# UCL-CCS/SCEMa

Hardware: AMD Instinct MI355X
Metric: stress_evals_per_sec (higher is better)
Workload: dtype f64; 1 GPU; 576 x PE-10368 OPLS replicas per update(), 10+100 MD steps each (dt 2 fs, 300 K, lj/cut/coul/long 12/9 + PPPM 1e-4 + SHAKE + NVT), persistent per-QP state, replica equilibrated for 2000 steps before the timed region; force_field=opls, strain_set=balanced (load/unload: odd updates take the draw with the opposite sign), n_sims=576, atoms_per_replica=10368, sims_on_rank0=576, allgathers=0

## Files before the change

### include/scema_md.h

```cpp
#ifndef SCEMA_MD_H
#define SCEMA_MD_H

#include <stdint.h>

#ifdef __cplusplus
extern "C" {
#endif

#define SCEMA_MD_OK 0
#define SCEMA_MD_ERR_ARG 1
#define SCEMA_MD_ERR_NOSTATE 2
#define SCEMA_MD_ERR_DEVICE 3
#define SCEMA_MD_ERR_BOX 4
#define SCEMA_MD_ERR_IO 5
#define SCEMA_MD_ERR_OVERFLOW 6

#define SCEMA_MD_NPART 8
#define SCEMA_MD_QP_NONE ((int32_t)0xFFFFFFFF)

typedef struct scema_md_engine scema_md_engine;

typedef struct {
  double cut_lj;
  double cut_coul;
// ... 142 lines not shown
                           double length[3], double stress[6], double stiff[36]);

typedef struct {
  int32_t nsteps_equil;
  double timestep_length;
  double temperature;
  int64_t seed;
} scema_md_equilparams;
int scema_md_equilibrate(scema_md_engine *e, const char *matid, int32_t replica, const scema_md_equilparams *p, double length[3],
                         double *info);

int scema_md_debug_minimize(scema_md_engine *e, int32_t qp_id, const char *matid, int32_t replica, double etol, double ftol,
                            int32_t maxiter, int32_t maxeval, double *info);
int scema_md_debug_run_nh(scema_md_engine *e, int32_t qp_id, const char *matid, int32_t replica, int32_t nsteps, double dt,
                          double t_start, double t_stop, int32_t npt, double p_target, double p_period, double *lavg);
int scema_md_debug_compute(scema_md_engine *e, int32_t qp_id, const char *matid, int32_t replica, int32_t use_shake,
                           double *f, double *energies, double *virials, double *info );
int scema_md_debug_skin_bands(scema_md_engine *e, int32_t pos, uint64_t *out, int32_t cap);
int scema_md_debug_rows(scema_md_engine *e, int32_t pos, int32_t *cnt, int32_t *rows, int64_t rows_cap, int32_t *info);
int scema_md_debug_run(scema_md_engine *e, int32_t qp_id, const char *matid, int32_t replica, int32_t nsteps,
                       double dt, double temperature, int32_t nvt, int32_t use_shake, const double *rates,
                       double *press_avg);

int scema_md_reax_configure(scema_md_engine *e, const char *ffield_path, const char *const *elements, int32_t n_elements,
                            double qeq_tol, double skin);
int scema_md_reax_activate(scema_md_engine *e, int32_t on);
int scema_md_reax_set(scema_md_engine *e, int32_t exact_gradient, int32_t terms, int32_t qeq_maxiter);
int scema_md_reax_concurrency(scema_md_engine *e, int32_t halves, int32_t overlap);
int scema_md_batch_split(scema_md_engine *e, int32_t on);
int scema_md_get_concurrency(const scema_md_engine *e, int32_t *out);
int scema_md_pppm_tiling(scema_md_engine *e, int32_t mode, int32_t lds_bytes);
int scema_md_pppm_binning(scema_md_engine *e, int32_t mode);
long long scema_md_pppm_binned_launches(const scema_md_engine *e);
int scema_md_pppm_paths(const scema_md_engine *e, int32_t out[8]);
int scema_md_pppm_tile_shape(const int32_t grid[3], int32_t lds_bytes, int32_t which , int32_t out[4]);
int scema_md_pppm_plan_count(const scema_md_engine *e);
int scema_md_reax_debug_compute(scema_md_engine *e, int32_t qp_id, const char *matid, int32_t replica, double *f, double *eparts,
                                double *virial, double *q, double *info);
int scema_md_reax_stats(const scema_md_engine *e, double *out);

int scema_md_sw_configure(scema_md_engine *e, const char *matid, const char *sw_path, const char *const *elements, int32_t n_elements,
                          int32_t energy_unit, double skin);
int scema_md_sw_debug_compute(scema_md_engine *e, int32_t qp_id, const char *matid, int32_t replica, double *f, double *e2, double *e3,
                              double *virial, double *info);
int scema_md_sw_read_params(const char *sw_path, const char *const *elements, int32_t n_elements, int32_t energy_unit, int32_t *n_kept,
                            int32_t *type_map, double *values, char *errbuf, int32_t errcap);

int scema_md_tersoff_configure(scema_md_engine *e, const char *matid, const char *path, const char *const *elements, int32_t n_elements,
                               int32_t energy_unit, double skin);
int scema_md_tersoff_debug_compute(scema_md_engine *e, int32_t qp_id, const char *matid, int32_t replica, double *f, double *e_rep,
                                   double *e_att, double *virial, double *info);
int scema_md_tersoff_read_params(const char *path, const char *const *elements, int32_t n_elements, int32_t energy_unit, int32_t *n_kept,
                                 int32_t *type_map, double *values, char *errbuf, int32_t errcap);

int scema_md_tersoff_mod_configure(scema_md_engine *e, const char *matid, const char *path, const char *const *elements, int32_t n_elements,
                                   int32_t energy_unit, double skin);
int scema_md_tersoff_mod_debug_compute(scema_md_engine *e, int32_t qp_id, const char *matid, int32_t replica, double *f, double *e_rep,
                                       double *e_att, double *virial, double *info);
int scema_md_tersoff_zbl_configure(scema_md_engine *e, const char *matid, const char *path, const char *const *elements, int32_t n_elements,
                                   int32_t energy_unit, double skin);
int scema_md_tersoff_zbl_debug_compute(scema_md_engine *e, int32_t qp_id, const char *matid, int32_t replica, double *f, double *e_rep,
                                       double *e_att, double *virial, double *info);
int scema_md_tersoff_mod_read_params(const char *path, const char *const *elements, int32_t n_elements, int32_t energy_unit, int32_t *n_kept,
                                     int32_t *type_map, double *values, char *errbuf, int32_t errcap);
int scema_md_tersoff_zbl_read_params(const char *path, const char *const *elements, int32_t n_elements, int32_t energy_unit, int32_t *n_kept,
                                     int32_t *type_map, double *values, char *errbuf, int32_t errcap);
// ... 89 lines not shown
```

### scema_amd/capi.py

```python
from __future__ import annotations

import ctypes as C
import os

import numpy as np

_HERE = os.path.dirname(os.path.abspath(__file__))
LIB_PATH = os.path.join(_HERE, os.environ.get("SCEMA_MD_LIB") or ("libscema_md_asan.so" if os.environ.get("SCEMA_SANITIZE") == "1" else "libscema_md.so"))

NPART = 8
PARTS = ["lj", "coul", "bond", "angle", "dihedral", "improper", "kspace", "shake"]
QP_NONE = -1

SYMBOLS = [
    "scema_md_default_params", "scema_md_create", "scema_md_destroy", "scema_md_last_error",
    "scema_md_register_replica", "scema_md_load_replica_file", "scema_md_write_replica_file",
    "scema_md_load_lammps_data", "scema_md_convert_lammps_data",
    "scema_md_probe_lammps_restart", "scema_md_read_lammps_restart_atoms", "scema_md_load_lammps_restart",
    "scema_md_convert_lammps_restart", "scema_md_write_lammps_restart",
    "scema_md_strain_batch", "scema_md_strain", "scema_md_local_stress_device_ptr",
    "scema_md_local_stress_count", "scema_md_local_result_doubles", "scema_md_copy_local_stress", "scema_md_scatter_gathered", "scema_md_settle_update", "scema_md_has_state", "scema_md_get_state",
    "scema_md_set_state", "scema_md_drop_state", "scema_md_save_state_file", "scema_md_load_state_file", "scema_md_save_state_lammps",
    "scema_md_init_material", "scema_md_debug_compute", "scema_md_debug_run", "scema_md_debug_skin_bands", "scema_md_debug_rows", "scema_md_get_profile", "scema_md_env_overrides",
    "scema_md_comm_unique_id", "scema_md_comm_init_rccl", "scema_md_comm_init_host", "scema_md_comm_destroy",
    "scema_md_comm_world", "scema_md_comm_rank", "scema_md_comm_stats", "scema_md_comm_handshakes", "scema_md_state_owner", "scema_md_last_plan",
    "scema_plan_dir_create", "scema_plan_dir_destroy", "scema_plan_update", "scema_md_kspace_setup",
    "scema_md_save_state_dump", "scema_md_replica_natoms", "scema_md_save_replica_file", "scema_md_equilibrate", "scema_md_debug_minimize", "scema_md_debug_run_nh",
    "scema_md_reax_configure", "scema_md_reax_activate", "scema_md_reax_set", "scema_md_reax_concurrency", "scema_md_batch_split", "scema_md_get_concurrency", "scema_md_pppm_plan_count", "scema_md_pppm_tiling", "scema_md_pppm_binning", "scema_md_pppm_binned_launches", "scema_md_pppm_paths", "scema_md_pppm_tile_shape", "scema_md_unsettled_updates", "scema_md_reax_debug_compute", "scema_md_reax_stats", "scema_md_box_fma_tflops",
    "scema_md_sw_configure", "scema_md_sw_debug_compute", "scema_md_sw_read_params",
    "scema_md_tersoff_configure", "scema_md_tersoff_debug_compute", "scema_md_tersoff_read_params",
    "scema_md_eam_configure", "scema_md_eam_debug_compute", "scema_md_eam_read_setfl",
    "scema_md_tersoff_mod_configure", "scema_md_tersoff_mod_debug_compute", "scema_md_tersoff_mod_read_params",
    "scema_md_tersoff_zbl_configure", "scema_md_tersoff_zbl_debug_compute", "scema_md_tersoff_zbl_read_params",
    "scema_md_vashishta_configure", "scema_md_vashishta_debug_compute", "scema_md_vashishta_read_params",
    "scema_md_adp_configure", "scema_md_adp_debug_compute", "scema_md_adp_read_setfl",
    "scema_md_edip_configure", "scema_md_edip_debug_compute", "scema_md_edip_read_params",
    "scema_md_meam_spline_configure", "scema_md_meam_spline_debug_compute", "scema_md_meam_spline_read_params", "scema_md_meam_spline_eval",
    "scema_md_born_dsf_configure", "scema_md_born_dsf_debug_compute", "scema_md_born_dsf_read_params", "scema_md_born_dsf_eval",
    "scema_md_born_long_configure", "scema_md_born_long_debug_compute", "scema_md_born_long_read_params", "scema_md_born_long_eval",
    "scema_md_born_long_kvectors",
]
COMM_ID_BYTES = 128
HOST_ALLGATHER_FN = C.CFUNCTYPE(C.c_int, C.c_void_p, C.c_void_p, C.c_void_p, C.c_int64)
HOST_SEND_FN = C.CFUNCTYPE(C.c_int, C.c_void_p, C.c_void_p, C.c_int64, C.c_int32)
HOST_RECV_FN = C.CFUNCTYPE(C.c_int, C.c_void_p, C.c_void_p, C.c_int64, C.c_int32)


class EquilParams(C.Structure):
    _fields_ = [("nsteps_equil", C.c_int32), ("timestep_length", C.c_double), ("temperature", C.c_double), ("seed", C.c_int64)]


class Params(C.Structure):
    _fields_ = [("cut_lj", C.c_double), ("cut_coul", C.c_double), ("skin", C.c_double), ("neigh_delay", C.c_int32),
                ("kspace_accuracy", C.c_double), ("shake_tol", C.c_double), ("shake_maxiter", C.c_int32),
                ("shake_mass", C.c_double), ("t_period", C.c_double), ("t_chain", C.c_int32), ("device", C.c_int32),
                ("max_batch", C.c_int32), ("profile", C.c_int32), ("kspace_style", C.c_int32)]


_P = C.c_void_p


# ... 365 lines not shown
        arr = (C.c_char_p * len(elements))(*[e.encode() for e in elements])
        self._chk(lib().scema_md_reax_configure(self.h, ffield.encode(), arr, C.c_int32(len(elements)), C.c_double(qeq_tol), C.c_double(skin)))

    def reax_activate(self, on: bool = True):
        self._chk(lib().scema_md_reax_activate(self.h, C.c_int32(1 if on else 0)))

    def reax_set(self, exact_gradient: int = -1, terms: int = -1, qeq_maxiter: int = -1):
        self._chk(lib().scema_md_reax_set(self.h, C.c_int32(exact_gradient), C.c_int32(terms), C.c_int32(qeq_maxiter)))

    def reax_concurrency(self, halves: int = -1, overlap: int = -1):
        self._chk(lib().scema_md_reax_concurrency(self.h, C.c_int32(halves), C.c_int32(overlap)))

    def unsettled_updates(self) -> int:
        lib().scema_md_unsettled_updates.restype = C.c_int64
        return int(lib().scema_md_unsettled_updates(self.h))

    def batch_split(self, on: int = -1):
        self._chk(lib().scema_md_batch_split(self.h, C.c_int32(on)))

    def pppm_plan_count(self) -> int:
        lib().scema_md_pppm_plan_count.restype = C.c_int
        return int(lib().scema_md_pppm_plan_count(self.h))

    def pppm_tiling(self, mode: int = -1, lds_bytes: int = -1):
        self._chk(lib().scema_md_pppm_tiling(self.h, C.c_int32(mode), C.c_int32(lds_bytes)))

    def pppm_binning(self, mode: int = -1):
        self._chk(lib().scema_md_pppm_binning(self.h, C.c_int32(mode)))

    def pppm_binned_launches(self) -> int:
        lib().scema_md_pppm_binned_launches.restype = C.c_longlong
        return int(lib().scema_md_pppm_binned_launches(self.h))

    def pppm_paths(self) -> dict:
        out = (C.c_int32 * 8)()
        self._chk(lib().scema_md_pppm_paths(self.h, out))
        return dict(spread=int(out[0]), force=int(out[1]), spread_tiles=(int(out[2]), int(out[3])), force_tiles=(int(out[4]), int(out[5])),
                    lds_bytes=int(out[6]), mode=int(out[7]))

    def concurrency(self) -> dict:
        out = (C.c_int32 * 3)()
        self._chk(lib().scema_md_get_concurrency(self.h, out))
        return dict(split=int(out[0]), reax_halves=int(out[1]), reax_overlap=int(out[2]))

    def reax_compute(self, matid, replica, qp=QP_NONE):
        n = self._natoms[(matid, replica)]
        f = np.zeros((n, 3)); e = np.zeros(len(REAX_PARTS)); w = np.zeros(6); q = np.zeros(n); info = np.zeros(6)
        self._chk(lib().scema_md_reax_debug_compute(self.h, C.c_int32(qp), matid.encode(), C.c_int32(replica), _p(f), _p(e), _p(w), _p(q), _p(info)))
        return dict(f=f, e=dict(zip(REAX_PARTS, e)), w=w, q=q, maxneigh_seen=int(info[0]), maxnb=int(info[1]), maxbd=int(info[2]),
                    qeq_iters=int(info[3]), image_search=int(info[4]), maxbonds_seen=int(info[5]))

    def _row_configure(self, symbol, matid, path, elements, energy_unit, skin):
        arr = (C.c_char_p * len(elements))(*[e.encode() for e in elements])
        self._chk(getattr(lib(), symbol)(self.h, matid.encode(), path.encode(), arr, C.c_int32(len(elements)), C.c_int32(energy_unit), C.c_double(skin)))

    def _row_compute(self, symbol, matid, replica, qp, ea_key, eb_key, count_key):
        n = self.natoms(matid, replica)
        f = np.zeros((n, 3)); ea = C.c_double(0.0); eb = C.c_double(0.0); w = np.zeros(6); info = np.zeros(4)
        self._chk(getattr(lib(), symbol)(self.h, C.c_int32(qp), matid.encode(), C.c_int32(replica), _p(f), C.byref(ea), C.byref(eb), _p(w), _p(info)))
        return {"f": f, ea_key: ea.value, eb_key: eb.value, "w": w, "maxrow": int(info[0]), "rowcap": int(info[1]), "npairs": int(info[2]),
                count_key: int(info[3])}

    def sw_configure(self, matid: str, sw_path: str, elements=("Si",), energy_unit: int = 0, skin: float = -1.0):
        self._row_configure("scema_md_sw_configure", matid, sw_path, elements, energy_unit, skin)

    def sw_compute(self, matid, replica, qp=QP_NONE):
# ... 433 lines not shown
```

### scema_amd/csrc/engine/engine.h

```cpp
#pragma once
#include <hip/hip_runtime.h>
#include <rccl/rccl.h>

#include <algorithm>
#include <cmath>
#include <cstdarg>
#include <cstdio>
#include <cstdlib>
#include <chrono>
#include <thread>
#include <cstring>
#include <ctime>
#include <array>
#include <atomic>
#include <functional>
#include <map>
#include <memory>
#include <sstream>
#include <fstream>
#include <string>
#include <vector>

#include "../../../include/scema_md.h"
#include "host/reax_ffield.h"
// ... 270 lines not shown
struct scema_md_engine {
  scema_md_params p;
  hipStream_t stream = nullptr;
  double skin_extra_fixed = 0.0;
  bool skin_adapt = false;
  hipStream_t stream2 = nullptr;
  hipStream_t stream3 = nullptr;
  hipEvent_t ev_up = nullptr;
  bool split_streams = true;
  hipEvent_t ev_fork = nullptr, ev_join = nullptr;
  bool rx_qeq_failed = false;
  long long rx_precond_fallbacks = 0;
  bool rx_precond = true;
  int rx_halves = 2, rx_overlap = 1;
  struct RxPart { hipStream_t main = nullptr, side = nullptr; hipEvent_t ev[4] = {nullptr, nullptr, nullptr, nullptr}; };
  std::vector<RxPart> rx_parts;
  std::vector<hipEvent_t> md_part_done;
  hipStream_t rx_side1 = nullptr;
  hipEvent_t rx_side1_ev[4] = {nullptr, nullptr, nullptr, nullptr};
  hipEvent_t row_fork = nullptr;
  std::map<std::string, std::unique_ptr<Topo>> topos;
  std::map<std::string, std::unique_ptr<State>> states;
  std::vector<std::unique_ptr<Slot>> slots;
  DevBuf d_sims, d_sc, d_local_stress, d_kpack, d_minptr, d_boxpair, d_pppm, d_copytab;
  std::vector<MdkCopy> h_copytab;
  DevBuf d_zerotab, d_rxstat;
  std::vector<MdkZero> h_zerotab;
  std::vector<long long> h_rxstat;
  std::vector<std::unique_ptr<DevBuf>> bak_x, bak_v;
  int pppm_tile_mode = 1, pppm_lds_bytes = 0;
  int pppm_paths[8] = {0, 0, 0, 0, 0, 0, 0, 1};
  int pppm_bin_mode = 2;
  long long pppm_binned_launches = 0;
  std::map<std::array<int, 6>, hipfftHandle> pppm_plans;
  std::vector<int> h_kpack;
  int local_stress_count = 0;
  std::vector<SimDev> h_sims;
  std::vector<SimScalars> h_sc;
  std::vector<hipEvent_t> ev_pool;
  Profile prof;
  std::string err;
  double neigh_grow = 1.0;
  double jtab_grow = 1.0;
  int overflow_bits = 0;
  double overflow_need_j = 1.0, overflow_need_row = 1.0;
  long long unsettled_updates = 0;
  bool rx_ready = false, reax_active = false;
  int rx_stamp = 0;
  RxParams rx_host;
  std::vector<int> rx_type_map;
  DevBuf d_rxparams, d_rxviews;
  std::vector<RxView> h_rxviews;
  double rx_skin = 0.75, rx_qeq_tol = 1e-6;
  int rx_qeq_maxiter = 200, rx_terms = 31;
  bool rx_sym = true;
  long long rx_qeq_iters = 0, rx_qeq_solves = 0, rx_qeq_slow = 0;
  int rx_qeq_launch_cold = 48;
  int rx_qeq_launch = 32;
  bool rx_qeq_launch_pinned = false;
  std::map<std::string, std::unique_ptr<RowMaterial>> row_mats;
  long long row_stamp = 0;
  DevBuf d_rowviews;
  std::vector<RowView> h_rowviews;
  DevBuf d_eamviews;
  std::vector<EamView> h_eamviews;
  DevBuf d_blviews;
// ... 171 lines not shown
```

### scema_amd/csrc/engine/engine_core.cpp

```cpp
#include <algorithm>
#include "engine.h"
#include "../md_env.h"

namespace scema_eng {

int fail(scema_md_engine *e, int code, const char *fmt, ...) {
  char buf[1024];
  va_list ap;
  va_start(ap, fmt);
  vsnprintf(buf, sizeof buf, fmt, ap);
  va_end(ap);
  if (e) e->err = buf;
  return code;
}

std::string topo_key(const char *matid, int replica) { return std::string(matid ? matid : "") + "_" + std::to_string(replica); }
std::string state_key(int qp, const char *matid, int replica) { return std::to_string(qp) + "." + topo_key(matid, replica); }

}

namespace scema_eng {
double event_union_ms(const std::vector<hipEvent_t> &ev, size_t n) {
  if (n == 0) return 0.0;
  std::vector<std::pair<float, float>> iv(n);
  for (size_t l = 0; l < n; l++) {
    float a = 0.f, b = 0.f;
    if (hipEventElapsedTime(&a, ev[0], ev[2 * l]) != hipSuccess || hipEventElapsedTime(&b, ev[0], ev[2 * l + 1]) != hipSuccess) return 0.0;
    iv[l] = {a, b};
  }
  std::sort(iv.begin(), iv.end());
  double total = 0.0;
  float lo = iv[0].first, hi = iv[0].second;
  for (size_t l = 1; l < n; l++) {
    if (iv[l].first > hi) { total += hi - lo; lo = iv[l].first; hi = iv[l].second; }
    else hi = std::max(hi, iv[l].second);
  }
  return total + (hi - lo);
}
}

namespace {
struct EnvSwitch { const char *name, *what; };
const EnvSwitch k_env[] = {
    {"SCEMA_MD_SPLIT", "0: never run a launch group of 9 simulations and more as part batches on streams of their own"},
    {"SCEMA_MD_PARTS", "2-4: this many part batches for every launch group that is split, if it has 2 replicas per part (default: by the size of the group, engine_run.cpp)"},
    {"SCEMA_MD_ONE_STREAM", "no side stream (bonded / k-space chain beside the pair kernel)"},
    {"SCEMA_MD_KEEP_LIST", "0: the sampling run of an evaluation rebuilds its neighbour rows at its start even where those of the straining run still hold"},
    {"SCEMA_MD_SKIN_BANDS", "0: the pair kernel walks every listed entry of a row on every step (default: the skin part of a row only as far as its cluster's and the replica's displacement bounds allow a pair inside the cutoff; results do not depend on it)"},
    {"SCEMA_MD_SKIN_EXTRA", "list skin = params.skin + this many Angstrom (results do not depend on it)"},
    {"SCEMA_MD_SKIN_ADAPT", "1: per-state adaptation of the extra skin from the rebuild interval (round-1 behaviour)"},
    {"SCEMA_MD_PPPM_SOLVE_WIDE", "1 / 0: the in-LDS PPPM solve with 1 024 threads and three LDS grids / 512 threads and two (default: by batch size)"},
    {"SCEMA_MD_PPPM_SOLVE_TWO", "0 / 1: the in-LDS PPPM solve of the 1 024-thread shape as one / two workgroups per replica, one per transform back (default: two for batches under 8 replicas)"},
    {"SCEMA_MD_PPPM_PADX", "0: the LDS grid of the PPPM spreading kernel without the five pad points per x row (an address addition per stencil point instead of a constant offset)"},
    {"SCEMA_MD_PPPM_BINNED", "0 / 1: the charge assignment of meshes kept whole in LDS never / wherever eligible as k_pppm_bins + k_pppm_spread_binned, atoms grouped by nearest grid point (default: by launch size and atoms per grid point)"},
    {"SCEMA_MD_PPPM_FFT", "hipFFT for every PPPM grid (default: grids of up to 2 900 points are solved in LDS)"},
    {"SCEMA_MD_FUSED_TAIL", "0 / 1: force assembly + SHAKE + second kick as three kernels / as k_finish (default: by batch size)"},
    {"SCEMA_MD_BONDED_SIDE", "0: the bonded kernel of a small batch always on the main stream behind the pair kernel (default: behind the PPPM chain on the side stream on steps without a new influence function)"},
    {"SCEMA_MD_SMALL_BATCH_MAX", "largest batch that takes the cell grid with the most cells instead of the largest cells (default: launch groups of up to 31 replicas that run whole, i.e. not as part batches)"},
    {"SCEMA_MD_REBUILD_TOGETHER", "0 / 1: every replica rebuilds its neighbour rows on its own trigger / the replicas of a launch rebuild together as soon as one asks for it (default: together in launches of fewer than 128 replicas)"},
    {"SCEMA_MD_CELL_BUILD", "0: cell binning as k_bin + k_cell_scan + k_cell_fill instead of the one-launch k_cell_build"},
    {"SCEMA_MD_ROW_CELLS", "0 / 1: the neighbour rows of the row potentials never through cells (the N^2 build for every replica) / through cells wherever the geometry allows it, whatever the size (default: for no replica -- no measured size gains in the update time, DESIGN.md 7m; rows and results do not depend on it)"},
    {"SCEMA_MD_POLY_TOL", "fit target of the real-space Ewald polynomial (default 2e-13); parity tolerances assume the default"},
    {"SCEMA_REAX_DROP_DSBO2", "ReaxFF valence-angle gradient without the dSBO2 term, as USER-REAXC is believed to compute it"},
    {"SCEMA_MD_RX_ITEM_LDS", "0 (test hook): the ReaxFF angle and torsion items add forces and dE/dDelta to the work set with device-wide atomics instead of through a workgroup's LDS tables (replicas too large for the tables do)"},
    {"SCEMA_MD_RX_NEAR_FULL", "1 (test hook): the ReaxFF near rows hold every pair within the 5 A bond cutoff + skin instead of the pairs within reach of their type pair's bond order"},
    {"SCEMA_REAX_SKIN", "ReaxFF list skin in Angstrom"},
    {"SCEMA_REAX_HALVES", "number of part batches a ReaxFF batch runs as, each on its own stream (default 2; 0 or 1: one sequence of launches)"},
    {"SCEMA_REAX_OVERLAP", "0: the bond-order chain of the ReaxFF force stage on the same stream as the charge chain instead of next to it"},
    {"SCEMA_REAX_QEQ_PRECOND", "0: the conjugate gradients of the charge equilibration with the Jacobi preconditioner of fix qeq/reax instead of the bonded-pattern approximate inverse"},
    {"SCEMA_REAX_QEQ_SYM", "0: the matrix of the charge equilibration as full rows (every pair in both rows) instead of each pair once in its owner's row"},
    {"SCEMA_REAX_QEQ_ZLDS", "0: the matrix sweep of the charge equilibration gathers through the caches instead of from an LDS copy"},
    {"SCEMA_REAX_QEQ_LAUNCH", "conjugate-gradient iterations issued as launches per charge solve (default: adaptive)"},
    {"SCEMA_MD_NEIGH_GROW0", "start with undersized neighbour capacities: overflow -> restore -> regrow"},
    {"SCEMA_MD_NEIGH_EXACT", "1: every list build tests its candidates in FP64 at the exact list radius; 0: none does (default: the first build of a run)"},
    {"SCEMA_MD_TEST_FAIL_INCOMING", "rank on which the allocation of a state that migrates in fails (-1: on whichever rank receives one); the failure must reach every rank through the handshake"},
    {"SCEMA_MD_TEST_FAIL_MIGRATE", "<what>[:<rank>] -- an injected failure of the exchange of replica states: dbox / upload (before the handshake: every rank ends the call, nothing is posted), enqueue / group / hostcopy (after it: the exchange is completed, the error travels in the status word of the stress all-gather)"},
    {"SCEMA_MD_TEST_SELF_MOVE", "1 (RCCL, one rank): every simulation that continues from a state held here receives it through ncclSend / ncclRecv from this very rank"},
    {"SCEMA_MD_TEST_QEQ_PRECOND_FAILS", "1: a ReaxFF run whose charge solve uses the approximate-inverse preconditioner reports that it did not converge (the evaluation must come back from its one retry with the Jacobi preconditioner)"},
    {"SCEMA_MD_QCAP16", "capacity of k_neigh_build's group lists in sixteenths of the table: small values force the whole-table walk"},
    {"SCEMA_MD_RX_COL32", "32-bit column indices in the ReaxFF charge matrix whatever the replica size"},
    {"SCEMA_MD_RX_NB_ONCE", "0: the both-ends ReaxFF non-bonded kernel"},
    {"SCEMA_MD_RX_ITEMCAP", "capacity of the work-item lists of the ReaxFF angle and torsion kernels: small values force their in-place path"},
    {"SCEMA_MD_TIMING", "per-chunk wall times and the PAIR_TIMING / PAIR_COUNT counters on stderr"},
};
}

const char *scema_env(const char *name) {
// ... 155 lines not shown
```

### scema_amd/csrc/engine/engine_reax.cpp

```cpp
#include "engine.h"
#include "../md_env.h"

namespace scema_eng {


#define RXSET(dst, src) dst = (decltype(dst))(src)
static int ensure_rx_slot(scema_md_engine *e, RxSlot &r, int n, int npad, int maxnb, int maxbd, int maxnbn, bool col16) {
  if (npad > r.cap_pad) {
    HIPCHK(r.nb_cnt.ensure((size_t)npad * 4));
    HIPCHK(r.bd_cnt.ensure((size_t)npad * 4));
    HIPCHK(r.deltap.ensure((size_t)npad * 8));
    HIPCHK(r.total_bo.ensure((size_t)npad * 8));
    HIPCHK(r.cd_delta.ensure((size_t)npad * 8));
    HIPCHK(r.hd.ensure((size_t)npad * 8));
    HIPCHK(r.q.ensure((size_t)npad * 8));
    HIPCHK(r.s.ensure((size_t)npad * 8));
    HIPCHK(r.t.ensure((size_t)npad * 8));
    HIPCHK(r.s_hist.ensure(4 * (size_t)npad * 8));
    HIPCHK(r.t_hist.ensure(3 * (size_t)npad * 8));
    HIPCHK(r.qwork.ensure(10 * (size_t)npad * 8));
    HIPCHK(r.qpart.ensure((10 * (size_t)((npad + 255) / 256) + 2 * (size_t)(npad / RX_SWR + 1)) * 8));
    HIPCHK(r.pm_len.ensure((size_t)npad * 4));
    HIPCHK(r.pm_col.ensure((size_t)RX_PM_MAX * npad * 4));
    HIPCHK(r.pm_raw.ensure((size_t)RX_PM_MAX * npad * 8));
// ... 346 lines not shown
  if (halves >= 0) e->rx_halves = std::min(halves, 8);
  if (overlap >= 0) e->rx_overlap = overlap != 0;
  return SCEMA_MD_OK;
}
int scema_md_batch_split(scema_md_engine *e, int32_t on) {
  if (!e) return SCEMA_MD_ERR_ARG;
  if (on >= 0) e->split_streams = on != 0;
  return SCEMA_MD_OK;
}
int scema_md_get_concurrency(const scema_md_engine *e, int32_t *out) {
  if (!e || !out) return SCEMA_MD_ERR_ARG;
  out[0] = e->split_streams ? 1 : 0;
  out[1] = e->rx_halves;
  out[2] = e->rx_overlap ? 1 : 0;
  return SCEMA_MD_OK;
}
int scema_md_pppm_tiling(scema_md_engine *e, int32_t mode, int32_t lds_bytes) {
  if (!e) return SCEMA_MD_ERR_ARG;
  if (mode < -1 || mode > 1) return fail(e, SCEMA_MD_ERR_ARG, "scema_md_pppm_tiling: mode %d (1 tiled kernels, 0 the kernels without LDS, -1 keeps)", mode);
  const int least = 2 * 8, most = 160 * 1024;
  if (lds_bytes < -1 || (lds_bytes > 0 && (lds_bytes < least || lds_bytes > most)))
    return fail(e, SCEMA_MD_ERR_ARG, "scema_md_pppm_tiling: an LDS budget of %d bytes (%d .. %d, 0 the device default, -1 keeps)", lds_bytes, least, most);
  if (mode >= 0) e->pppm_tile_mode = mode;
  if (lds_bytes >= 0) e->pppm_lds_bytes = lds_bytes;
  return SCEMA_MD_OK;
}
int scema_md_pppm_binning(scema_md_engine *e, int32_t mode) {
  if (!e) return SCEMA_MD_ERR_ARG;
  if (mode < -1 || mode > 2) return fail(e, SCEMA_MD_ERR_ARG, "scema_md_pppm_binning: mode %d (0 off, 1 wherever eligible, 2 by the launch policy, -1 keeps)", mode);
  if (mode >= 0) e->pppm_bin_mode = mode;
  return SCEMA_MD_OK;
}
long long scema_md_pppm_binned_launches(const scema_md_engine *e) { return e ? e->pppm_binned_launches : -(long long)SCEMA_MD_ERR_ARG; }
int scema_md_pppm_paths(const scema_md_engine *e, int32_t out[8]) {
  if (!e || !out) return SCEMA_MD_ERR_ARG;
  for (int k = 0; k < 8; k++) out[k] = e->pppm_paths[k];
  return SCEMA_MD_OK;
}
int scema_md_pppm_tile_shape(const int32_t grid[3], int32_t lds_bytes, int32_t which, int32_t out[4]) {
  if (!grid || !out || grid[0] < 1 || grid[1] < 1 || grid[2] < 1 || lds_bytes < 0 || which < 0 || which > 1) return SCEMA_MD_ERR_ARG;
  const PppmTile t = pppm_tile_shape(grid[0], grid[1], grid[2], lds_bytes > 0 ? lds_bytes : (long long)mdk_pppm_lds_limit(), which);
  out[0] = t.by; out[1] = t.bz; out[2] = t.ty; out[3] = t.tz;
  return SCEMA_MD_OK;
}
int scema_md_pppm_plan_count(const scema_md_engine *e) { return e ? (int)e->pppm_plans.size() : -SCEMA_MD_ERR_ARG; }
int scema_md_reax_set(scema_md_engine *e, int32_t exact_gradient, int32_t terms, int32_t qeq_maxiter) {
  if (!e || !e->rx_ready) return fail(e, SCEMA_MD_ERR_ARG, "no ReaxFF force field loaded");
  HIPCHK(hipSetDevice(e->p.device));
  if (exact_gradient >= 0) {
    e->rx_host.lammps_dsbo2 = exact_gradient ? 0 : 1;
    HIPCHK(hipMemcpyAsync(e->d_rxparams.p, &e->rx_host, sizeof(RxParams), hipMemcpyHostToDevice, e->stream));
    HIPCHK(hipStreamSynchronize(e->stream));
  }
  if (terms >= 0) e->rx_terms = terms;
  if (qeq_maxiter > 0) e->rx_qeq_maxiter = qeq_maxiter;
  return SCEMA_MD_OK;
}
int scema_md_reax_debug_compute(scema_md_engine *e, int32_t qp_id, const char *matid, int32_t replica, double *f, double *eparts, double *virial,
                                double *q, double *info) {
  if (!e) return SCEMA_MD_ERR_ARG;
  if (!e->rx_ready) return fail(e, SCEMA_MD_ERR_ARG, "no ReaxFF force field loaded");
  HIPCHK(hipSetDevice(e->p.device));
  State *s = nullptr;
  std::unique_ptr<State> tmp;
  int rc = debug_state(e, qp_id, matid, replica, &s, tmp);
  if (rc) return rc;
// ... 48 lines not shown
```

### scema_amd/csrc/engine/engine_run.cpp

```cpp
#include "engine.h"
#include "../md_env.h"

namespace scema_eng {

static int padded_slots(int natoms, int ncells) { return (natoms + (MD_CLUSTER - 1) * ncells + 255) / 256 * 256; }

int ensure_slot(scema_md_engine *e, Slot &sl, int natoms, int maxneigh, int ncells, int nk, int capj) {
  const int npad = padded_slots(natoms, ncells);
  if (natoms > sl.cap_atoms || npad > sl.cap_pad) {
    HIPCHK(sl.f.ensure(3 * (size_t)natoms * 8));
    HIPCHK(sl.slot_of.ensure((size_t)natoms * 4));
    HIPCHK(sl.fs.ensure(3 * (size_t)npad * 8));
    HIPCHK(sl.fb.ensure(3 * (size_t)npad * 8));
    HIPCHK(sl.virb.ensure(((size_t)natoms / BT_OWNERS + 2) * 6 * 8));
    HIPCHK(sl.tile_order.ensure((size_t)npad * 4));
    HIPCHK(sl.wrapn.ensure(3 * (size_t)natoms * 4));
    HIPCHK(sl.xhold.ensure(3 * (size_t)natoms * 8));
    HIPCHK(sl.cell_of.ensure((size_t)natoms * 4));
    HIPCHK(sl.ckey.ensure((size_t)natoms * 4));
    HIPCHK(sl.slot_tmp.ensure((size_t)npad * 4));
    HIPCHK(sl.xbak.ensure(3 * (size_t)natoms * 8));
    HIPCHK(sl.vbak.ensure(3 * (size_t)natoms * 8));
    HIPCHK(sl.xq.ensure((size_t)npad * 32));
    HIPCHK(sl.stype.ensure((size_t)npad * 4));
// ... 439 lines not shown
  const std::array<int, 6> key = {pg[0], pg[1], pg[2], batch, sk, L.maxgrid};
  auto it = e->pppm_plans.find(key);
  if (it == e->pppm_plans.end()) {
    hipfftHandle h;
    int n[3] = {pg[2], pg[1], pg[0]};
    if (hipfftPlanMany(&h, 3, n, n, 1, L.maxgrid, n, 1, L.maxgrid, HIPFFT_Z2Z, batch) != HIPFFT_SUCCESS)
      return fail(e, SCEMA_MD_ERR_DEVICE, "hipfftPlanMany failed for a %d x %d x %d grid, batch %d", pg[0], pg[1], pg[2], batch);
    it = e->pppm_plans.emplace(key, h).first;
  }
  plan = it->second;
  return SCEMA_MD_OK;
}

int OplsRun::pppm_stage(hipStream_t st, int pos0, int na, bool new_box, int add) {
  if (L.maxgrid <= 0 || na <= 0) return SCEMA_MD_OK;
  const SimDev *Dp = D + pos0;
  bool &clean = pppm_clean[part_of(parts, pos0)];
  const int maxgridp = L.padx_ok ? L.maxgridp : 0;
  const int sp_path = mdk_pppm_spread_path(L.maxgrid, maxgridp, &L.tl), fo_path = mdk_pppm_force_path(L.maxgrid, &L.tl);
  {
    const int paths[8] = {sp_path, fo_path, sp_path == 1 ? L.tl.sp_ty : 1, sp_path == 1 ? L.tl.sp_tz : 1, fo_path == 1 ? L.tl.fo_ty : 1,
                          fo_path == 1 ? L.tl.fo_tz : 1, L.tl.budget, L.tl.mode};
    std::memcpy(e->pppm_paths, paths, sizeof paths);
  }
  if (sp_path == 1 || fo_path == 1) mdk_pppm_keys(st, Dp, na, L.maxatoms);
  static const int binned_env = scema_env("SCEMA_MD_PPPM_BINNED") ? (atoi(scema_env("SCEMA_MD_PPPM_BINNED")) != 0 ? 1 : 0) : -1;
  const int bin_mode = binned_env >= 0 ? binned_env : e->pppm_bin_mode;
  PppmLaunch tl = L.tl;
  if (bin_mode != 0 && mdk_pppm_binned_ok(L.maxgrid, maxgridp, &L.tl)) {
    const PppmBinPolicy bp;
    tl.binned = bin_mode == 1 || (na >= bp.min_replicas && (double)L.sum_charged >= bp.min_per_point * (double)L.sum_grid) ? 1 : 0;
  }
  if (tl.binned) e->pppm_binned_launches += 1;
  mdk_pppm_spread(st, Dp, na, L.maxgrid, L.maxatoms, clean ? 1 : 0, maxgridp, &tl);
  clean = false;
  if (pol.pppm_in_lds) {
    if (new_box) mdk_pppm_gf(st, Dp, na, L.maxgrid);
    mdk_pppm_solve(st, Dp, na, L.maxgrid, L.maxdims);
    clean = true;
    mdk_pppm_force(st, Dp, na, L.maxgrid, L.maxatoms, add, 1, &L.tl);
    return SCEMA_MD_OK;
  }
  auto transform = [&](bool fields, int dir) -> int {
    for (const auto &run : pppm_runs) {
      if (run.first + run.second <= pos0 || run.first >= pos0 + na) continue;
      const SimDev &S0 = e->h_sims[run.first];
      if (S0.pg[0] == 0) continue;
      hipfftHandle plan;
      const int rc = pppm_plan(S0.pg, (fields ? 3 : 1) * run.second, st, plan);
      if (rc) return rc;
      double *g = fields ? S0.pfield : S0.pgrid;
      if (hipfftSetStream(plan, st) != HIPFFT_SUCCESS || hipfftExecZ2Z(plan, (hipfftDoubleComplex *)g, (hipfftDoubleComplex *)g, dir) != HIPFFT_SUCCESS)
        return fail(e, SCEMA_MD_ERR_DEVICE, "hipfftExecZ2Z failed");
    }
    return SCEMA_MD_OK;
  };
  int rc = transform(false, HIPFFT_FORWARD);
  if (rc) return rc;
  if (new_box) mdk_pppm_gf(st, Dp, na, L.maxgrid);
  mdk_pppm_poisson(st, Dp, na, L.maxgrid);
  if ((rc = transform(true, HIPFFT_BACKWARD))) return rc;
  mdk_pppm_force(st, Dp, na, L.maxgrid, L.maxatoms, add, 0, &L.tl);
  return SCEMA_MD_OK;
}

int OplsRun::pppm_fork(hipStream_t st, int pos0, int na, bool new_box, bool with_bonded) {
  if (!pol.pppm_side) return SCEMA_MD_OK;
  HIPCHK(hipEventRecord(e->ev_fork, st));
  HIPCHK(hipStreamWaitEvent(e->stream2, e->ev_fork, 0));
  const int rc = pppm_stage(e->stream2, pos0, na, new_box, 0);
  if (rc) return rc;
  if (with_bonded) mdk_bonded(e->stream2, D + pos0, na, L.maxbt, L.maxloc, L.maxcoef, 0);
  HIPCHK(hipEventRecord(e->ev_join, e->stream2));
  return SCEMA_MD_OK;
}

hipError_t OplsRun::force_stage(hipStream_t st, const SimDev *Dh, int na, bool side, int bparts, int pairvir, bool pppm_ahead) {
  hipError_t rc;
  if (side) {
    if ((rc = hipEventRecord(e->ev_fork, st)) != hipSuccess) return rc;
    if ((rc = hipStreamWaitEvent(e->stream2, e->ev_fork, 0)) != hipSuccess) return rc;
    mdk_ewald_recip(e->stream2, Dh, na, L.maxk, L.mmax, L.maxgrp);
    if ((rc = hipEventRecord(e->ev_join, e->stream2)) != hipSuccess) return rc;
  }
  mdk_bonded(st, Dh, na, L.maxbt, L.maxloc, L.maxcoef, bparts);
  if (side) {
    if ((rc = hipStreamWaitEvent(st, e->ev_join, 0)) != hipSuccess) return rc;
  } else {
    mdk_ewald_recip(st, Dh, na, L.maxk, L.mmax, L.maxgrp);
  }
  if (pppm_ahead) {
    if ((rc = hipStreamWaitEvent(st, e->ev_join, 0)) != hipSuccess) return rc;
  }
  mdk_ewald_force(st, Dh, na, L.maxatoms, pairvir, pppm_ahead ? 1 : 0);
  return hipSuccess;
// ... 263 lines not shown
```

### scema_amd/csrc/md_pppm.h

```cpp
#pragma once
#include <hip/hip_runtime.h>
struct SimDev;
size_t mdk_pppm_lds_limit();
struct PppmLaunch {
  int budget = 0, mode = 1;
  int sp_ty = 0, sp_tz = 0, sp_tiles = 0, fo_ty = 0, fo_tz = 0, fo_tiles = 0;
  size_t sp_lds = 0, fo_lds = 0;
  int binned = 0;
};
struct PppmBinPolicy { int min_replicas = 72; double min_per_point = 2.0; };
int mdk_pppm_binned_ok(int maxgrid, int maxgridp, const PppmLaunch *tl);
int mdk_pppm_spread_path(int maxgrid, int maxgridp, const PppmLaunch *tl);
int mdk_pppm_force_path(int maxgrid, const PppmLaunch *tl);
void mdk_pppm_keys(hipStream_t st, const SimDev *d, int ns, int maxatoms);
int mdk_pppm_spread(hipStream_t st, const SimDev *d, int ns, int maxgrid, int maxatoms, int zeroed, int maxgridp = 0, const PppmLaunch *tl = nullptr);
int mdk_pppm_solve_max();
void mdk_pppm_solve(hipStream_t st, const SimDev *d, int ns, int maxgrid, int maxdims);
void mdk_pppm_gf(hipStream_t st, const SimDev *d, int ns, int maxgrid);
void mdk_pppm_poisson(hipStream_t st, const SimDev *d, int ns, int maxgrid);
int mdk_pppm_force(hipStream_t st, const SimDev *d, int ns, int maxgrid, int maxatoms, int add, int real_fields = 0, const PppmLaunch *tl = nullptr);
```

### scema_amd/csrc/md_pppm.hip

```cpp
#include <hip/hip_runtime.h>

#include "md_device.h"
#include "md_env.h"
#include "md_pppm.h"
#include "md_pppm_tile.h"
#include "md_types.h"

#include <algorithm>
#include <cstdlib>

static inline dim3 grid2(int nx, int ns) { return dim3((unsigned)nx, (unsigned)ns, 1); }
static inline int cdiv(int a, int b) { return (a + b - 1) / b; }

#define PP_ORDER 5
#define PP_TPB 1024
#define PP_SOLVE_MAX 2900

static_assert(PP_ORDER == 5, "the blending polynomials below are those of order 5");
__device__ __forceinline__ int pppm_nearest(double u) { return (int)floor(u + 0.5); }
__device__ __forceinline__ void pppm_blend(double s, double (&w)[PP_ORDER]) {
  const double r = 1.0 - s;
  const double s2 = s * s, r2 = r * r;
  constexpr double q = 1.0 / 24.0;
  w[4] = q * (s2 * s2);
// ... 571 lines not shown
    const double qa = S.q[a];
    if (qa == 0.0) {
      if (!add) { S.f[3 * a] = 0.0; S.f[3 * a + 1] = 0.0; S.f[3 * a + 2] = 0.0; }
      continue;
    }
    double l0, l1, l2;
    atom_lamda(S, b, a, l0, l1, l2);
    double wx[PP_ORDER], wy[PP_ORDER], wz[PP_ORDER];
    int gx[PP_ORDER], gy[PP_ORDER], gz[PP_ORDER];
    pppm_wrap(pppm_weights(l0 * nx, wx), nx, gx);
    pppm_wrap(pppm_weights(l1 * ny, wy), ny, gy);
    pppm_wrap(pppm_weights(l2 * nz, wz), nz, gz);
    double fx = 0.0, fy = 0.0, fz = 0.0;
#pragma unroll
    for (int c = 0; c < PP_ORDER; c++) {
#pragma unroll
      for (int bb = 0; bb < PP_ORDER; bb++) {
        const double zy = wz[c] * wy[bb];
        const int row = (gz[c] * ny + gy[bb]) * nx;
        double rx = 0.0, ry = 0.0, rz = 0.0;
#pragma unroll
        for (int k = 0; k < PP_ORDER; k++) {
          const int g = row + gx[k];
          if (LDS) { rx = fma(wx[k], s_grid[g], rx); ry = fma(wx[k], s_grid[NG + g], ry); rz = fma(wx[k], s_grid[2 * NG + g], rz); }
          else if (REALF) { const double *fr = (const double *)S.pfield; rx = fma(wx[k], fr[g], rx); ry = fma(wx[k], fr[gs + g], ry); rz = fma(wx[k], fr[2 * gs + g], rz); }
          else { rx = fma(wx[k], ex[g].x, rx); ry = fma(wx[k], ey[g].x, ry); rz = fma(wx[k], ez[g].x, rz); }
        }
        fx = fma(zy, rx, fx); fy = fma(zy, ry, fy); fz = fma(zy, rz, fz);
      }
    }
    const double qf = MD_QQRD2E * qa;
    if (add) { S.f[3 * a] += qf * fx; S.f[3 * a + 1] += qf * fy; S.f[3 * a + 2] += qf * fz; }
    else { S.f[3 * a] = qf * fx; S.f[3 * a + 1] = qf * fy; S.f[3 * a + 2] = qf * fz; }
  }
}


#define PP_KEY_Y(key) ((key) & 0xffff)
#define PP_KEY_Z(key) (((key) >> 16) & 0x7fff)
__global__ __launch_bounds__(256) void k_pppm_keys(const SimDev *sims) {
  const SimDev &S = sims[blockIdx.y];
  if (S.pg[0] == 0) return;
  const int ny = S.pg[1], nz = S.pg[2], a = blockIdx.x * 256 + threadIdx.x;
  if (a >= S.natoms) return;
  BoxD b;
  box_derive(S.sc->box, b);
  box_uniform(b);
  double l0, l1, l2;
  atom_lamda(S, b, a, l0, l1, l2);
  const int iy = pmod(pppm_nearest(l1 * ny), ny), iz = pmod(pppm_nearest(l2 * nz), nz);
  pppm_keys_of(S)[a] = iy | (iz << 16) | (S.q[a] == 0.0 ? (int)0x80000000 : 0);
}
struct PppmBrick { int y0, z0, byc, bzc, hy, hz; };
__device__ __forceinline__ bool pppm_brick(int nx, int ny, int nz, int budget, int which, PppmBrick &B) {
  const PppmTile t = pppm_tile_shape(nx, ny, nz, budget, which);
  const int tile = (int)blockIdx.x;
  if (tile >= t.ty * t.tz) return false;
  const int tzi = tile / t.ty, tyi = tile - tzi * t.ty;
  B.y0 = tyi * t.by; B.z0 = tzi * t.bz;
  B.byc = min(t.by, ny - B.y0); B.bzc = min(t.bz, nz - B.z0);
  B.hy = t.by < ny ? 4 : 0; B.hz = t.bz < nz ? 4 : 0;
  return true;
}
__device__ __forceinline__ int pppm_rel(int a, int b, int d, int n) {
  const int v = a - b + d;
  return v < 0 ? v + n : (v >= n ? v - n : v);
// ... 244 lines not shown
void mdk_pppm_poisson(hipStream_t st, const SimDev *d, int ns, int maxgrid) { hipLaunchKernelGGL(k_pppm_poisson, grid2(cdiv(maxgrid, 256), ns), dim3(256), 0, st, d); }
int mdk_pppm_force(hipStream_t st, const SimDev *d, int ns, int maxgrid, int maxatoms, int add, int real_fields, const PppmLaunch *tl) {
  const size_t lds = 3 * (size_t)maxgrid * sizeof(double);
  const int path = mdk_pppm_force_path(maxgrid, tl);
  if (path == 1) {
    const size_t tlds = tl->fo_lds;
    static size_t optin_tab[16] = {0};
    size_t &optin = lds_optin_slot(optin_tab);
    if (tlds > 64 * 1024 && tlds > optin) {
      (void)hipFuncSetAttribute((const void *)k_pppm_force_tiled<PP_TPB, false>, hipFuncAttributeMaxDynamicSharedMemorySize, (int)tlds);
      (void)hipFuncSetAttribute((const void *)k_pppm_force_tiled<PP_TPB, true>, hipFuncAttributeMaxDynamicSharedMemorySize, (int)tlds);
      optin = tlds;
    }
    const dim3 g = grid2(tl->fo_tiles, ns);
    if (tlds <= 36 * 1024) {
      if (real_fields) hipLaunchKernelGGL((k_pppm_force_tiled<256, true>), g, dim3(256), tlds, st, d, tl->budget, add);
      else hipLaunchKernelGGL((k_pppm_force_tiled<256, false>), g, dim3(256), tlds, st, d, tl->budget, add);
    } else {
      if (real_fields) hipLaunchKernelGGL((k_pppm_force_tiled<PP_TPB, true>), g, dim3(PP_TPB), tlds, st, d, tl->budget, add);
      else hipLaunchKernelGGL((k_pppm_force_tiled<PP_TPB, false>), g, dim3(PP_TPB), tlds, st, d, tl->budget, add);
    }
    return path;
  }
  if (path == 2) {
    if (real_fields) hipLaunchKernelGGL((k_pppm_force<false, true>), grid2(cdiv(maxatoms, 256), ns), dim3(256), 0, st, d, cdiv(maxatoms, 256), add);
    else hipLaunchKernelGGL((k_pppm_force<false, false>), grid2(cdiv(maxatoms, 256), ns), dim3(256), 0, st, d, cdiv(maxatoms, 256), add);
    return path;
  }
  static size_t optin_tab[16] = {0};
  size_t &optin = lds_optin_slot(optin_tab);
  if (lds > 64 * 1024 && lds > optin) {
    (void)hipFuncSetAttribute((const void *)k_pppm_force<true, false>, hipFuncAttributeMaxDynamicSharedMemorySize, (int)lds);
    (void)hipFuncSetAttribute((const void *)k_pppm_force<true, true>, hipFuncAttributeMaxDynamicSharedMemorySize, (int)lds);
    optin = lds;
  }
  const int split = pppm_split(ns, maxatoms);
  if (real_fields) hipLaunchKernelGGL((k_pppm_force<true, true>), grid2(split, ns), dim3(256), lds, st, d, split, add);
  else hipLaunchKernelGGL((k_pppm_force<true, false>), grid2(split, ns), dim3(256), lds, st, d, split, add);
  return path;
}
```

Measured before the change: 475.3 evals/s.

## Add binned PPPM force interpolation reusing field stencil across atoms of a grid point

Adds k_pppm_force_binned, which walks the per-grid-point atom lists built by the binned charge assignment. Each lane loads the 5x5x5 field stencil around one grid point from LDS once and applies it to up to M atoms, instead of every atom reading its own stencil. The intent is to cut LDS reads in the interpolation step. In exchange it adds an extra pass to zero forces on uncharged atoms, more register pressure from the per-atom weight arrays, and load imbalance across items with uneven atom counts. It is enabled by default whenever the spread is binned and the whole-grid LDS force path is selected.

```diff
diff --git a/include/scema_md.h b/include/scema_md.h
--- a/include/scema_md.h
+++ b/include/scema_md.h
@@ -198,6 +198,8 @@
 int scema_md_pppm_tiling(scema_md_engine *e, int32_t mode, int32_t lds_bytes);
 int scema_md_pppm_binning(scema_md_engine *e, int32_t mode);
 long long scema_md_pppm_binned_launches(const scema_md_engine *e);
+int scema_md_pppm_binned_force(scema_md_engine *e, int32_t mode);
+long long scema_md_pppm_binned_force_launches(const scema_md_engine *e);
 int scema_md_pppm_paths(const scema_md_engine *e, int32_t out[8]);
 int scema_md_pppm_tile_shape(const int32_t grid[3], int32_t lds_bytes, int32_t which , int32_t out[4]);
 int scema_md_pppm_plan_count(const scema_md_engine *e);
diff --git a/scema_amd/capi.py b/scema_amd/capi.py
--- a/scema_amd/capi.py
+++ b/scema_amd/capi.py
@@ -26,7 +26,7 @@
     "scema_md_comm_world", "scema_md_comm_rank", "scema_md_comm_stats", "scema_md_comm_handshakes", "scema_md_state_owner", "scema_md_last_plan",
     "scema_plan_dir_create", "scema_plan_dir_destroy", "scema_plan_update", "scema_md_kspace_setup",
     "scema_md_save_state_dump", "scema_md_replica_natoms", "scema_md_save_replica_file", "scema_md_equilibrate", "scema_md_debug_minimize", "scema_md_debug_run_nh",
-    "scema_md_reax_configure", "scema_md_reax_activate", "scema_md_reax_set", "scema_md_reax_concurrency", "scema_md_batch_split", "scema_md_get_concurrency", "scema_md_pppm_plan_count", "scema_md_pppm_tiling", "scema_md_pppm_binning", "scema_md_pppm_binned_launches", "scema_md_pppm_paths", "scema_md_pppm_tile_shape", "scema_md_unsettled_updates", "scema_md_reax_debug_compute", "scema_md_reax_stats", "scema_md_box_fma_tflops",
+    "scema_md_reax_configure", "scema_md_reax_activate", "scema_md_reax_set", "scema_md_reax_concurrency", "scema_md_batch_split", "scema_md_get_concurrency", "scema_md_pppm_plan_count", "scema_md_pppm_tiling", "scema_md_pppm_binning", "scema_md_pppm_binned_launches", "scema_md_pppm_binned_force", "scema_md_pppm_binned_force_launches", "scema_md_pppm_paths", "scema_md_pppm_tile_shape", "scema_md_unsettled_updates", "scema_md_reax_debug_compute", "scema_md_reax_stats", "scema_md_box_fma_tflops",
     "scema_md_sw_configure", "scema_md_sw_debug_compute", "scema_md_sw_read_params",
     "scema_md_tersoff_configure", "scema_md_tersoff_debug_compute", "scema_md_tersoff_read_params",
     "scema_md_eam_configure", "scema_md_eam_debug_compute", "scema_md_eam_read_setfl",
@@ -458,6 +458,13 @@
         lib().scema_md_pppm_binned_launches.restype = C.c_longlong
         return int(lib().scema_md_pppm_binned_launches(self.h))
 
+    def pppm_binned_force(self, mode: int = -1):
+        self._chk(lib().scema_md_pppm_binned_force(self.h, C.c_int32(mode)))
+
+    def pppm_binned_force_launches(self) -> int:
+        lib().scema_md_pppm_binned_force_launches.restype = C.c_longlong
+        return int(lib().scema_md_pppm_binned_force_launches(self.h))
+
     def pppm_paths(self) -> dict:
         out = (C.c_int32 * 8)()
         self._chk(lib().scema_md_pppm_paths(self.h, out))
diff --git a/scema_amd/csrc/engine/engine.h b/scema_amd/csrc/engine/engine.h
--- a/scema_amd/csrc/engine/engine.h
+++ b/scema_amd/csrc/engine/engine.h
@@ -326,6 +326,8 @@
   int pppm_paths[8] = {0, 0, 0, 0, 0, 0, 0, 1};
   int pppm_bin_mode = 2;
   long long pppm_binned_launches = 0;
+  int pppm_bin_force_mode = 1;
+  long long pppm_binned_force_launches = 0;
   std::map<std::array<int, 6>, hipfftHandle> pppm_plans;
   std::vector<int> h_kpack;
   int local_stress_count = 0;
diff --git a/scema_amd/csrc/engine/engine_core.cpp b/scema_amd/csrc/engine/engine_core.cpp
--- a/scema_amd/csrc/engine/engine_core.cpp
+++ b/scema_amd/csrc/engine/engine_core.cpp
@@ -53,6 +53,7 @@
     {"SCEMA_MD_PPPM_SOLVE_TWO", "0 / 1: the in-LDS PPPM solve of the 1 024-thread shape as one / two workgroups per replica, one per transform back (default: two for batches under 8 replicas)"},
     {"SCEMA_MD_PPPM_PADX", "0: the LDS grid of the PPPM spreading kernel without the five pad points per x row (an address addition per stencil point instead of a constant offset)"},
     {"SCEMA_MD_PPPM_BINNED", "0 / 1: the charge assignment of meshes kept whole in LDS never / wherever eligible as k_pppm_bins + k_pppm_spread_binned, atoms grouped by nearest grid point (default: by launch size and atoms per grid point)"},
+    {"SCEMA_MD_PPPM_BINNED_FORCE", "0 / 1: the interpolation behind a binned charge assignment (field grids staged whole) never / always as k_pppm_force_binned, a lane reading the field around a grid point once for the atoms of an item (default 1)"},
     {"SCEMA_MD_PPPM_FFT", "hipFFT for every PPPM grid (default: grids of up to 2 900 points are solved in LDS)"},
     {"SCEMA_MD_FUSED_TAIL", "0 / 1: force assembly + SHAKE + second kick as three kernels / as k_finish (default: by batch size)"},
     {"SCEMA_MD_BONDED_SIDE", "0: the bonded kernel of a small batch always on the main stream behind the pair kernel (default: behind the PPPM chain on the side stream on steps without a new influence function)"},
diff --git a/scema_amd/csrc/engine/engine_reax.cpp b/scema_amd/csrc/engine/engine_reax.cpp
--- a/scema_amd/csrc/engine/engine_reax.cpp
+++ b/scema_amd/csrc/engine/engine_reax.cpp
@@ -402,6 +402,13 @@
   return SCEMA_MD_OK;
 }
 long long scema_md_pppm_binned_launches(const scema_md_engine *e) { return e ? e->pppm_binned_launches : -(long long)SCEMA_MD_ERR_ARG; }
+int scema_md_pppm_binned_force(scema_md_engine *e, int32_t mode) {
+  if (!e) return SCEMA_MD_ERR_ARG;
+  if (mode < -1 || mode > 1) return fail(e, SCEMA_MD_ERR_ARG, "scema_md_pppm_binned_force: mode %d (0 never, 1 whenever the step's lists exist, -1 keeps)", mode);
+  if (mode >= 0) e->pppm_bin_force_mode = mode;
+  return SCEMA_MD_OK;
+}
+long long scema_md_pppm_binned_force_launches(const scema_md_engine *e) { return e ? e->pppm_binned_force_launches : -(long long)SCEMA_MD_ERR_ARG; }
 int scema_md_pppm_paths(const scema_md_engine *e, int32_t out[8]) {
   if (!e || !out) return SCEMA_MD_ERR_ARG;
   for (int k = 0; k < 8; k++) out[k] = e->pppm_paths[k];
diff --git a/scema_amd/csrc/engine/engine_run.cpp b/scema_amd/csrc/engine/engine_run.cpp
--- a/scema_amd/csrc/engine/engine_run.cpp
+++ b/scema_amd/csrc/engine/engine_run.cpp
@@ -495,13 +495,16 @@
     tl.binned = bin_mode == 1 || (na >= bp.min_replicas && (double)L.sum_charged >= bp.min_per_point * (double)L.sum_grid) ? 1 : 0;
   }
   if (tl.binned) e->pppm_binned_launches += 1;
+  static const int binned_force_env = scema_env("SCEMA_MD_PPPM_BINNED_FORCE") ? (atoi(scema_env("SCEMA_MD_PPPM_BINNED_FORCE")) != 0 ? 1 : 0) : -1;
+  tl.binned_force = tl.binned && fo_path == 0 && (binned_force_env >= 0 ? binned_force_env : e->pppm_bin_force_mode) != 0 ? 1 : 0;
+  if (tl.binned_force) e->pppm_binned_force_launches += 1;
   mdk_pppm_spread(st, Dp, na, L.maxgrid, L.maxatoms, clean ? 1 : 0, maxgridp, &tl);
   clean = false;
   if (pol.pppm_in_lds) {
     if (new_box) mdk_pppm_gf(st, Dp, na, L.maxgrid);
     mdk_pppm_solve(st, Dp, na, L.maxgrid, L.maxdims);
     clean = true;
-    mdk_pppm_force(st, Dp, na, L.maxgrid, L.maxatoms, add, 1, &L.tl);
+    mdk_pppm_force(st, Dp, na, L.maxgrid, L.maxatoms, add, 1, &tl);
     return SCEMA_MD_OK;
   }
   auto transform = [&](bool fields, int dir) -> int {
@@ -523,7 +526,7 @@
   if (new_box) mdk_pppm_gf(st, Dp, na, L.maxgrid);
   mdk_pppm_poisson(st, Dp, na, L.maxgrid);
   if ((rc = transform(true, HIPFFT_BACKWARD))) return rc;
-  mdk_pppm_force(st, Dp, na, L.maxgrid, L.maxatoms, add, 0, &L.tl);
+  mdk_pppm_force(st, Dp, na, L.maxgrid, L.maxatoms, add, 0, &tl);
   return SCEMA_MD_OK;
 }
 
diff --git a/scema_amd/csrc/md_pppm.h b/scema_amd/csrc/md_pppm.h
--- a/scema_amd/csrc/md_pppm.h
+++ b/scema_amd/csrc/md_pppm.h
@@ -7,6 +7,7 @@
   int sp_ty = 0, sp_tz = 0, sp_tiles = 0, fo_ty = 0, fo_tz = 0, fo_tiles = 0;
   size_t sp_lds = 0, fo_lds = 0;
   int binned = 0;
+  int binned_force = 0;
 };
 struct PppmBinPolicy { int min_replicas = 72; double min_per_point = 2.0; };
 int mdk_pppm_binned_ok(int maxgrid, int maxgridp, const PppmLaunch *tl);
diff --git a/scema_amd/csrc/md_pppm.hip b/scema_amd/csrc/md_pppm.hip
--- a/scema_amd/csrc/md_pppm.hip
+++ b/scema_amd/csrc/md_pppm.hip
@@ -627,6 +627,103 @@
     const double qf = MD_QQRD2E * qa;
     if (add) { S.f[3 * a] += qf * fx; S.f[3 * a + 1] += qf * fy; S.f[3 * a + 2] += qf * fz; }
     else { S.f[3 * a] = qf * fx; S.f[3 * a + 1] = qf * fy; S.f[3 * a + 2] = qf * fz; }
+  }
+}
+
+#ifndef PP_BINF_M
+#define PP_BINF_M 2
+#endif
+template <int M, bool REALF>
+__global__ __launch_bounds__(256) void k_pppm_force_binned(const SimDev *sims, int split, int add) {
+  static_assert(PP_BIN_M % M == 0, "an item is taken in passes of M atoms");
+  const SimDev &S = sims[blockIdx.y];
+  const int nx = S.pg[0], ny = S.pg[1], nz = S.pg[2];
+  if (nx == 0) return;
+  const int NG = nx * ny * nz, nbx = nx + 1, natoms = S.natoms;
+  if (!add) {
+    int achunk = (natoms + split - 1) / split;
+    achunk = (achunk + 255) & ~255;
+    const int a0 = (int)blockIdx.x * achunk, a1 = min(natoms, a0 + achunk);
+    for (int a = a0 + (int)threadIdx.x; a < a1; a += 256)
+      if (S.q[a] == 0.0) { S.f[3 * a] = 0.0; S.f[3 * a + 1] = 0.0; S.f[3 * a + 2] = 0.0; }
+  }
+  const int MD_G *head = pppm_keys_of(S);
+  const int2 MD_G *items = (const int2 MD_G *)(head + 2);
+  const int MD_G *perm = head + 2 + 2 * (size_t)natoms;
+  const int nitems = head[0];
+  const int chunk = (nitems + split - 1) / split, i0 = (int)blockIdx.x * chunk, i1 = min(nitems, i0 + chunk);
+  if (i0 >= i1) return;
+  const size_t gs = (size_t)S.pgstride;
+  if (REALF) {
+    const double *fr = (const double *)S.pfield;
+    for (int k = threadIdx.x; k < NG; k += 256) { s_grid[k] = fr[k]; s_grid[NG + k] = fr[gs + k]; s_grid[2 * NG + k] = fr[2 * gs + k]; }
+  } else {
+    const double2 *ex = (const double2 *)S.pfield, *ey = ex + gs, *ez = ey + gs;
+    for (int k = threadIdx.x; k < NG; k += 256) { s_grid[k] = ex[k].x; s_grid[NG + k] = ey[k].x; s_grid[2 * NG + k] = ez[k].x; }
+  }
+  __syncthreads();
+  BoxD b;
+  box_derive(S.sc->box, b);
+  box_uniform(b);
+  for (int p0 = 0; p0 < PP_BIN_M; p0 += M) {
+  for (int it = i0 + (int)threadIdx.x; it < i1; it += 256) {
+    const int2 item = items[it];
+    const int bin = item.x & 0xffffff, nit = item.x >> 24;
+    if (p0 >= nit) continue;
+    const int rowb = bin / nbx, ix = bin - rowb * nbx, iz = rowb / ny, iy = rowb - iz * ny;
+    int gx[PP_ORDER], gy[PP_ORDER], gz[PP_ORDER];
+    pppm_wrap(ix, nx, gx); pppm_wrap(iy, ny, gy); pppm_wrap(iz, nz, gz);
+    {
+      const int n = min(nit - p0, M), first = item.y + p0;
+      int at[M];
+      double px[M], py[M], pz[M], qa[M];
+#pragma unroll
+      for (int j = 0; j < M; j++) at[j] = perm[first + min(j, n - 1)];
+#pragma unroll
+      for (int j = 0; j < M; j++) { px[j] = S.x[3 * at[j]]; py[j] = S.x[3 * at[j] + 1]; pz[j] = S.x[3 * at[j] + 2]; qa[j] = S.q[at[j]]; }
+      double wx[M][PP_ORDER], wy[M][PP_ORDER], wz[M][PP_ORDER];
+      double fx[M], fy[M], fz[M];
+#pragma unroll
+      for (int j = 0; j < M; j++) {
+        double l0, l1, l2;
+        pos_lamda(b, px[j], py[j], pz[j], l0, l1, l2);
+        pppm_blend(0.5 - ((double)ix - l0 * nx), wx[j]);
+        pppm_weights_at(l1 * ny, ny, iy, wy[j]); pppm_weights_at(l2 * nz, nz, iz, wz[j]);
+        fx[j] = 0.0; fy[j] = 0.0; fz[j] = 0.0;
+      }
+#pragma unroll
+      for (int c = 0; c < PP_ORDER; c++) {
+#pragma unroll
+        for (int bb = 0; bb < PP_ORDER; bb++) {
+          const int row = (gz[c] * ny + gy[bb]) * nx;
+          double ex[PP_ORDER], ey[PP_ORDER], ez[PP_ORDER];
+#pragma unroll
+          for (int k = 0; k < PP_ORDER; k++) {
+            const int g = row + gx[k];
+            ex[k] = s_grid[g]; ey[k] = s_grid[NG + g]; ez[k] = s_grid[2 * NG + g];
+          }
+#pragma unroll
+          for (int j = 0; j < M; j++) {
+            const double zy = wz[j][c] * wy[j][bb];
+            double rx = 0.0, ry = 0.0, rz = 0.0;
+#pragma unroll
+            for (int k = 0; k < PP_ORDER; k++) { rx = fma(wx[j][k], ex[k], rx); ry = fma(wx[j][k], ey[k], ry); rz = fma(wx[j][k], ez[k], rz); }
+            fx[j] = fma(zy, rx, fx[j]); fy[j] = fma(zy, ry, fy[j]); fz[j] = fma(zy, rz, fz[j]);
+          }
+#pragma unroll
+          for (int j = 0; j < M; j++) asm volatile("" : "+v"(fx[j]), "+v"(fy[j]), "+v"(fz[j]) : : "memory");
+        }
+      }
+#pragma unroll
+      for (int j = 0; j < M; j++) {
+        if (j >= n) continue;
+        const int a = at[j];
+        const double qf = MD_QQRD2E * qa[j];
+        if (add) { S.f[3 * a] += qf * fx[j]; S.f[3 * a + 1] += qf * fy[j]; S.f[3 * a + 2] += qf * fz[j]; }
+        else { S.f[3 * a] = qf * fx[j]; S.f[3 * a + 1] = qf * fy[j]; S.f[3 * a + 2] = qf * fz[j]; }
+      }
+    }
+  }
   }
 }
 
@@ -937,9 +1034,16 @@
   if (lds > 64 * 1024 && lds > optin) {
     (void)hipFuncSetAttribute((const void *)k_pppm_force<true, false>, hipFuncAttributeMaxDynamicSharedMemorySize, (int)lds);
     (void)hipFuncSetAttribute((const void *)k_pppm_force<true, true>, hipFuncAttributeMaxDynamicSharedMemorySize, (int)lds);
+    (void)hipFuncSetAttribute((const void *)k_pppm_force_binned<PP_BINF_M, false>, hipFuncAttributeMaxDynamicSharedMemorySize, (int)lds);
+    (void)hipFuncSetAttribute((const void *)k_pppm_force_binned<PP_BINF_M, true>, hipFuncAttributeMaxDynamicSharedMemorySize, (int)lds);
     optin = lds;
   }
   const int split = pppm_split(ns, maxatoms);
+  if (tl && tl->binned && tl->binned_force) {
+    if (real_fields) hipLaunchKernelGGL((k_pppm_force_binned<PP_BINF_M, true>), grid2(split, ns), dim3(256), lds, st, d, split, add);
+    else hipLaunchKernelGGL((k_pppm_force_binned<PP_BINF_M, false>), grid2(split, ns), dim3(256), lds, st, d, split, add);
+    return path;
+  }
   if (real_fields) hipLaunchKernelGGL((k_pppm_force<true, true>), grid2(split, ns), dim3(256), lds, st, d, split, add);
   else hipLaunchKernelGGL((k_pppm_force<true, false>), grid2(split, ns), dim3(256), lds, st, d, split, add);
   return path;
```

Result: no change. 478.2 evals/s, median of 6 (+0.6%).
